# teaghan/sky_embeddings

Measured on AMD Instinct MI355X. Metric: MAE pretrain images/sec (5x64x64, ViT-B), higher is better.
Workload: dtype f16; 1 GPU; mim_32.ini-as-BASELINE configs[1]: MAE ViT-Base/16, 5x64x64, mask_ratio=0.75, bs=256/GPU, AdamW+cosine, norm_pix mse; global_batch=256, parallelism=dp1, rccl_ranks=1, graph=True, adamw_in_wgrad_epilogue=True

## Files before the change

include/skyemb.h:

```cpp
#ifndef SKYEMB_H
#define SKYEMB_H

#include <stdint.h>

#ifdef __cplusplus
extern "C" {
#endif

#define SKYEMB_BF16 0
#define SKYEMB_F32 1
#define SKYEMB_F16 2

#define SKYEMB_KC 0
#define SKYEMB_RC 1

#define SKYEMB_ACT_NONE 0
#define SKYEMB_ACT_GELU 1
#define SKYEMB_ACT_DGELU 2

const char *skyemb_last_error(void);
int skyemb_version(void);
int skyemb_debug_skip(int mask);
#define SKYEMB_GEMM_COUNT_FALLBACK 0
#define SKYEMB_GEMM_COUNT_PIPE 1
// ... 45 lines not shown
    int32_t tile;
    int32_t class_mask;
    int32_t reserved;
} skyemb_gemm_group_info;
int64_t skyemb_gemm_group_blob_bytes(int n);
int skyemb_gemm_group_plan(const skyemb_gemm_args *args, int n, int tile, void *blob_host, int64_t blob_bytes,
                           skyemb_gemm_group_info *info);
int skyemb_gemm_group_launch(const void *blob_dev, const skyemb_gemm_group_info *info, void *stream);
typedef struct skyemb_adamw_desc {
    float *g_base, *p, *m, *v;
    void *p_lp;
    const float *hyper;
    int64_t n_decay;
    float beta1, beta2, eps, weight_decay, grad_scale;
    int32_t enabled;
} skyemb_adamw_desc;
int skyemb_gemm_group_plan_adamw(const skyemb_gemm_args *args, int n, int tile, const skyemb_adamw_desc *adamw, void *blob_host,
                                 int64_t blob_bytes, skyemb_gemm_group_info *info);
int skyemb_gemm_group_plan_side_adamw(const skyemb_gemm_args *args, int n, int tile, const skyemb_adamw_desc *adamw, int own_step,
                                      int64_t side_lo, int64_t side_hi, int side_blocks, void *blob_host, int64_t blob_bytes,
                                      skyemb_gemm_group_info *info);
typedef struct skyemb_ln_bwd_side {
    const void *dy;
    const float *x, *gamma, *mean, *rstd;
    const float *g_in;
    float *g_out;
    void *g_lp;
    float *part;
    int32_t M, D;
} skyemb_ln_bwd_side;
int skyemb_gemm_group_attach_ln_bwd(void *blob_host, int64_t blob_bytes, skyemb_gemm_group_info *info, const skyemb_ln_bwd_side *ln);

int skyemb_colsum(const void *X, int dtype, int64_t ldx, int M, int N, float *out, void *stream);

int skyemb_random_mask_from_noise(const float *noise, int B, int L, int keep, int64_t *ids_restore, float *mask,
                                  int32_t *ids_keep, int32_t *dec_dst, int32_t *dec_tab, int n_extra, void *stream);
int skyemb_simmim_mask_from_noise(const float *noise, const float *ratio_u, double max_ratio, int B, int C, int L, int grid, int p,
                                  float *out_mask, void *stream);

int skyemb_patch_gather(const float *imgs, const float *pmv, const int32_t *ids_keep, void *out, int dtype, int B,
                        int C, int H, int W, int p, int keep, float pixel_mean, float pixel_std, void *stream);

int skyemb_patch_gather_blend(const float *imgs, const float *pmv, const int32_t *ids_keep, const float *pixel_mask, void *out,
                              int dtype, int B, int C, int H, int W, int p, int keep, float pixel_mean, float pixel_std,
                              void *stream);
int skyemb_patch_gather_bwd_pmv_blend(const float *imgs, const int32_t *ids_keep, const float *pixel_mask, const float *drows,
                                      float *partial, float *dpmv, int B, int C, int H, int W, int p, int keep, void *stream);

int skyemb_radec_token_fwd(const float *ra_dec, const float *W0, const float *b0, const float *W1, const float *b1,
                           const float *pos_row, float *x, int64_t row_stride, int B, int D, float *sh, float *z, void *stream);
int skyemb_radec_token_bwd(const float *g, int64_t row_stride, const float *W1, const float *sh, const float *z, float *dz_ws,
                           float *dW0, float *db0, float *dW1, float *db1, int B, int D, void *stream);

int skyemb_patch_gather_bwd_pmv(const float *imgs, const int32_t *ids_keep, const float *drows, float *partial,
                                float *dpmv, int B, int C, int H, int W, int p, int keep, void *stream);

int skyemb_layernorm_fwd(const float *x, const float *gamma, const float *beta, void *y, float *y32, int dtype,
                         float *mean, float *rstd, int M, int D, float eps, void *stream);

int skyemb_layernorm_bwd_blocks(int M);
typedef struct {
    const float *part;
    float *dgamma, *dbeta;
    int32_t nblk, D;
} skyemb_ln_reduce_item;
int skyemb_layernorm_bwd_reduce_batch(const skyemb_ln_reduce_item *items, const int32_t *blocks, int n_blocks, void *stream);
int skyemb_layernorm_bwd(const void *dy, int dy_is_f32, int dtype, const float *x, const float *gamma,
                         const float *mean, const float *rstd, const float *g_in, float *g_out, void *g_lp,
                         float *part, float *dgamma, float *dbeta, int M, int D, void *stream);

#define SKYEMB_MHA_MAX_N 4098
int skyemb_mha_fwd(const void *qkv, void *out, int dtype, int B, int N, int H, int hd, void *stream);
int skyemb_mha_bwd(const void *qkv, const void *dout, void *dqkv, int dtype, int B, int N, int H, int hd,
                   void *stream);
#define SKYEMB_MHA_LDS 0
#define SKYEMB_MHA_STREAM 1
#define SKYEMB_MHA_MFMA_PACKED 2
#define SKYEMB_MHA_MFMA_SINGLE 3
#define SKYEMB_MHA_MFMA_STRIP 4
#define SKYEMB_MHA_MFMA_LONG 5
#define SKYEMB_MHA_SW_NO_MFMA 1
#define SKYEMB_MHA_SW_WPB1 2
#define SKYEMB_MHA_SW_WPB4 4
typedef struct {
    int32_t family;
    int32_t hd;
    int32_t waves;
    int32_t per_wave_floats, nheads;
    int32_t grid_x, grid_y, block;
    int64_t lds_bytes;
    int64_t lds_limit;
} skyemb_mha_plan_t;
int skyemb_mha_plan(int bwd, int dtype, int B, int N, int H, int hd, int switches, skyemb_mha_plan_t *out);

int skyemb_fill_mask_tokens(float *x, const float *mask, const float *mask_token, const float *dec_pos, int B,
                            int L, int Dd, int n_extra, void *stream);
int skyemb_gather_rows(const float *src, const int32_t *idx, float *out, void *out_lp, int dtype, int n_rows,
                       int D, void *stream);
int skyemb_rowsum_select(const float *src, int64_t ld, const float *sel, int row0, int inner, int outer_stride,
                         int n_rows, int D, float *partial, float *out, void *stream);

int skyemb_masked_patch_loss(const float *imgs, const float *pred, const float *mask, float *loss, void *dpred,
                             float *dpred32, int dtype, float *ws, int B, int C, int H, int W, int p, int extra,
                             float pixel_mean, float pixel_std, int norm_pix, int loss_l1, float dscale, void *stream);

int skyemb_simmim_pixel_loss(const float *imgs, const float *pred_tok, const float *pixel_mask, float *loss, void *dpred_tok,
                             int dtype, float *pred_img, float *ws, int B, int C, int H, int W, int p, int extra,
                             float pixel_mean, float pixel_std, int norm_pix, int loss_l1, int pooled, float dscale, void *stream);

int skyemb_set_scalars(float *dst, float a, float b, float c, float d, void *stream);
int skyemb_adamw(float *p, void *g, float *m, float *v, void *p_lp, int dtype, int64_t n, int64_t n_decay,
                 const float *hyper, float lr, float bc1, float bc2, float beta1, float beta2, float eps, float wd,
                 float grad_scale, int zero_grad, int grad_dtype, void *stream);
int skyemb_cast(const float *src, void *dst, int dtype, int64_t n, void *stream);
int skyemb_grad_probe(const void *g, int grad_dtype, int64_t n, uint32_t *state, void *stream);
int skyemb_adamw_guarded(float *p, void *g, float *m, float *v, void *p_lp, int dtype, int64_t n, int64_t n_decay,
                         const float *hyper, float lr, float bc1, float bc2, float beta1, float beta2, float eps, float wd,
                         float grad_scale, int zero_grad, int grad_dtype, const uint32_t *skip, void *stream);
typedef struct skyemb_adamw_group { float lr, bc1, bc2, beta1, beta2, eps, wd; int32_t decayed; } skyemb_adamw_group;
typedef struct skyemb_adamw_segment { int64_t offset, n; int32_t group, reserved; } skyemb_adamw_segment;
typedef struct skyemb_adamw_work { int64_t offset; int32_t n, group; } skyemb_adamw_work;
int skyemb_adamw_segments_limits(int32_t *max_groups, int32_t *chunk_elems, int32_t *max_grid);
int skyemb_adamw_segments_plan(const skyemb_adamw_segment *segs, int n_segs, int n_groups, int64_t buffer_n, void *table_host,
                               int64_t table_bytes, int64_t *need_bytes, int32_t *n_work);
int skyemb_adamw_segments(float *p, const float *g, float *m, float *v, void *p_lp, int dtype, const void *table_dev, int32_t n_work,
                          const skyemb_adamw_group *groups, int n_groups, float grad_scale, const uint32_t *skip, void *stream);

int skyemb_gather_rows_host(const void *src, int64_t row_bytes, const int64_t *idx, int64_t n, int64_t src_rows, void *dst,
                            int nthreads);
int skyemb_h5_unchunk_host(const void *file_base, int64_t file_bytes, const int64_t *chunk_addr, const int64_t *chunk_off,
                           int64_t nchunks, int rank, const int64_t *chunk_dims, const int64_t *dset_dims, int elem_size, void *dst,
                           int nthreads);
int skyemb_fits_decode_tiles_host(int codec, const void *base, int64_t base_bytes, const int64_t *off, const int64_t *len,
                                  const int64_t *npix, const int64_t *dst_off, int64_t ntiles, int bytepix, int blocksize, void *dst,
                                  int64_t dst_pixels, int nthreads);
int skyemb_fits_dequantise_tiles_host(const int32_t *q, const int64_t *q_off, const int64_t *y0, const int64_t *x0, const int64_t *h,
                                      const int64_t *w, const int64_t *table_row, int64_t ntiles, const double *zscale, const double *zzero,
                                      const int32_t *blank, const uint8_t *has_blank, const float *rand, int method, int zdither0,
                                      float *out, int64_t H, int64_t W, int big_endian_out, int nthreads);
int skyemb_tile_cutouts(const void *tile, const int *big_endian, int C, int H, int W, const int *h0, const int *w0, int n, int S,
                        float lo, float hi, int use_lo, int use_hi, float *out, void *stream);
int skyemb_clip_crop(const float *src, float *dst, int64_t n_planes, int Hs, int Ws, int size, float lo, float hi,
                     int use_lo, int use_hi, void *stream);

int skyemb_augment(const float *imgs, float *out, const float *params, const int32_t *nan_mask, const float *noise, int B, int C,
                   int S, int A, void *stream);

int skyemb_standardise(const float *x, const float *mu, const float *sigma, float *out, int64_t N, int D,
                       void *stream);
int skyemb_weighted_norms(const float *x, const float *w, float *norms, float *xw_out, int64_t N, int D,
                          void *stream);
int skyemb_cosine_topk_chunks(int64_t N, int Q, int D, int k);
int skyemb_cosine_topk(const float *tw, const float *qn, const float *bank, const float *xn, int Q, int64_t N,
                       int D, int k, float eps, int64_t idx_offset, int nchunks, const float *thr0, float *part_s,
                       int64_t *part_i, void *stream);
int skyemb_kth_largest_floor(const float *x, int Q, int S, int k, float *out, void *stream);
int skyemb_cosine_sample_floor(const float *tw, const float *qn, const float *sample, const float *sample_norms, int Q, int64_t S,
                               int D, int k, float eps, float *ws, float *floor_out, void *stream);
int skyemb_cosine_sample_floor_applicable(int Q, int64_t S, int D, int k);
int skyemb_topk_merge(const float *in_s, const int64_t *in_i, int Q, int nlists, int k, float *out_s,
                      int64_t *out_i, void *ws, void *stream);

int skyemb_topk_prefilter_applicable(int Q, int64_t N, int D, int k);
int64_t skyemb_topk_prefilter_ws_bytes(int Q, int D, int k);
int skyemb_topk_prefilter_ws_layout(int Q, int D, int k, int64_t *out, int n);
int64_t skyemb_bank16_bytes(int64_t N, int D);
// ... 223 lines not shown
```

sky_embeddings_amd/_lib.py:

```python
from __future__ import annotations

import ctypes
import os
import subprocess

import torch

_HERE = os.path.dirname(os.path.abspath(__file__))
SO_PATH = os.environ.get("SKYEMB_LIB") or os.path.join(_HERE, "libskyemb.so")
CSRC = os.path.join(_HERE, "csrc")

BF16, F32, F16 = 0, 1, 2
ABI_VERSION = 111
KC, RC = 0, 1
ACT_NONE, ACT_GELU, ACT_DGELU = 0, 1, 2
COMBINE_MIN, COMBINE_MEAN, COMBINE_MAX = 0, 1, 2
METRIC_MSE, METRIC_MAE = 1, 2
MHA_LDS, MHA_STREAM, MHA_MFMA_PACKED, MHA_MFMA_SINGLE, MHA_MFMA_STRIP, MHA_MFMA_LONG = range(6)
MHA_SW_NO_MFMA, MHA_SW_WPB1, MHA_SW_WPB4 = 1, 2, 4
PF_ROWS, PF_TOKENS, PF_TOKENS_MEAN = range(3)
PF_BANK_F32, PF_BANK_F16, PF_BANK_BF16 = range(3)
PF_LO_UNSET, PF_MAX_SLICES = 2, 6
PROBE_CHUNKS, PROBE_MAX_F, PROBE_MIN_K, PROBE_MAX_K = 32, 4096, 3, 16


class SkyembLibraryError(RuntimeError):
    pass


class SkyembError(RuntimeError):
    pass


c_i32, c_i64, c_f32, c_vp = ctypes.c_int32, ctypes.c_int64, ctypes.c_float, ctypes.c_void_p
c_f64 = ctypes.c_double


class GemmArgs(ctypes.Structure):
    _fields_ = [
        ("A", c_vp), ("B", c_vp), ("lda", c_i64), ("ldb", c_i64), ("a_layout", c_i32), ("b_layout", c_i32),
        ("M", c_i32), ("N", c_i32), ("K", c_i32), ("dtype", c_i32), ("alpha", c_f32),
        ("bias", c_vp), ("table", c_vp), ("tab_row", c_vp), ("ldt", c_i64), ("dst_row", c_vp),
        ("resid", c_vp), ("ldr", c_i64), ("aux", c_vp), ("ldaux", c_i64), ("act", c_i32),
        ("out_f32", c_vp), ("ldo32", c_i64), ("out", c_vp), ("ldo", c_i64), ("out2", c_vp), ("ldo2", c_i64),
        ("tile", c_i32), ("colsum_a", c_vp), ("ws", c_vp), ("ws_bytes", c_i64), ("split_k", c_i32), ("prefetch_wgs", c_i32),
        ("prefetch", c_vp), ("prefetch_bytes", c_i64),
    ]


class AdamwDesc(ctypes.Structure):
    _fields_ = [("g_base", c_vp), ("p", c_vp), ("m", c_vp), ("v", c_vp), ("p_lp", c_vp), ("hyper", c_vp), ("n_decay", c_i64),
                ("beta1", c_f32), ("beta2", c_f32), ("eps", c_f32), ("weight_decay", c_f32), ("grad_scale", c_f32), ("enabled", c_i32)]


class LnBwdSide(ctypes.Structure):
    _fields_ = [("dy", c_vp), ("x", c_vp), ("gamma", c_vp), ("mean", c_vp), ("rstd", c_vp), ("g_in", c_vp), ("g_out", c_vp), ("g_lp", c_vp),
                ("part", c_vp), ("M", c_i32), ("D", c_i32)]


class MhaPlan(ctypes.Structure):
    _fields_ = [("family", c_i32), ("hd", c_i32), ("waves", c_i32), ("per_wave_floats", c_i32), ("nheads", c_i32),
                ("grid_x", c_i32), ("grid_y", c_i32), ("block", c_i32), ("lds_bytes", c_i64), ("lds_limit", c_i64)]


class PrefilterRequest(ctypes.Structure):
    _fields_ = [("kind", c_i32), ("bank", c_i32), ("Q", c_i32), ("P", c_i32), ("D", c_i32), ("k", c_i32), ("N", c_i64), ("combine", c_i32),
                ("top_t", c_i32), ("has_thr0", c_i32), ("sel", c_i32), ("n_live", c_i32), ("last_live", c_i32), ("direct_sel", c_i32),
                ("lo", c_i32), ("eps", c_f32)]


class PrefilterSlice(ctypes.Structure):
    _fields_ = [("mode", c_i32), ("t0", c_i32), ("t1", c_i32), ("bucket", c_i32), ("tail", c_i32), ("tail_sel", c_i32), ("tail_pos", c_i32),
                ("final", c_i32)]


class PrefilterPlan(ctypes.Structure):
    _fields_ = [("use_lo", c_i32), ("cap", c_i32), ("T", c_i32), ("T_tail", c_i32), ("has_tail", c_i32), ("first", c_i32),
                ("first_rows", c_i32), ("direct_end", c_i32), ("ends", c_i32 * 6), ("sel", c_i32), ("bf", c_i32), ("tok", c_i32),
                ("cnt", c_i32), ("tok_word", c_i32), ("lgp", c_i32), ("fold", c_i32), ("top_t", c_i32), ("q_padded", c_i32),
                ("lds_stage1", c_i32), ("lds_close", c_i32), ("lds_rescore", c_i32), ("lds_stage1_limit", c_i32),
                ("lds_close_limit", c_i32), ("eps_a_f32", c_f32), ("gfac", c_f32), ("eps_a", c_f64), ("rows", c_i64), ("n_slices", c_i32),
                ("slice", PrefilterSlice * 6)]


class AdamwGroup(ctypes.Structure):
    _fields_ = [("lr", c_f32), ("bc1", c_f32), ("bc2", c_f32), ("beta1", c_f32), ("beta2", c_f32), ("eps", c_f32), ("wd", c_f32),
                ("decayed", c_i32)]


class AdamwSegment(ctypes.Structure):
    _fields_ = [("offset", c_i64), ("n", c_i64), ("group", c_i32), ("reserved", c_i32)]


class GemmGroupInfo(ctypes.Structure):
    _fields_ = [("total_blocks", c_i32), ("tile", c_i32), ("class_mask", c_i32), ("reserved", c_i32)]


PROTOTYPES = {
    "skyemb_last_error": (ctypes.c_char_p, []),
    "skyemb_version": (c_i32, []),
    "skyemb_debug_skip": (c_i32, [c_i32]),
    "skyemb_gemm_launch_counts": (c_i32, [c_vp, c_i32, c_i32]),
# ... 216 lines not shown
```

sky_embeddings_amd/csrc/attention.hip:

```cpp
#include "attention_plan.h"
#include "common.h"
#include <stdlib.h>

namespace {

__device__ __forceinline__ float dot4(const float4 a, const float4 b, float acc) {
    acc = fmaf(a.x, b.x, acc);
    acc = fmaf(a.y, b.y, acc);
    acc = fmaf(a.z, b.z, acc);
    return fmaf(a.w, b.w, acc);
}

template <typename T>
__device__ __forceinline__ void load_head(const T *__restrict__ src, int64_t row_stride, float *dst, int N, int hd,
                                          int pitch, float scale, int lane) {
    const int v4 = hd >> 2;
    for (int e = lane; e < N * v4; e += 64) {
        const int n = e / v4, d = (e - n * v4) << 2;
        const float4 x = load4<T>(src + (int64_t)n * row_stride + d);
        *(float4 *)&dst[n * pitch + d] = make_float4(x.x * scale, x.y * scale, x.z * scale, x.w * scale);
    }
}

__device__ __forceinline__ void scores_softmax(const float *qs, const float *k, float *P, int N, int NP, int hd, int pitch,
// ... 211 lines not shown
        for (int c = 0; c < SH_C; ++c) a[c] = 0.f;
        for (int j0 = 0; j0 < N; j0 += 64) {
            const int j = j0 + lane;
            float ds = 0.f;
            if (j < N) {
                const float s = dot_row<T>(ra, kb + (int64_t)j * rs, hd), dp = dot_row<T>(rb, vb + (int64_t)j * rs, hd);
                ds = __expf(s - lse_i) * (dp - d_i);
            }
            sa[lane] = ds;
            __builtin_amdgcn_wave_barrier();
            const int nj = N - j0 < 64 ? N - j0 : 64;
            for (int jj = 0; jj < nj; ++jj) {
                const float dsj = sa[jj];
                const T *kr = kb + (int64_t)(j0 + jj) * rs;
#pragma unroll
                for (int c = 0; c < SH_C; ++c)
                    if (lane + 64 * c < hd) a[c] = fmaf(dsj, to_f32<T>(kr[lane + 64 * c]), a[c]);
            }
            __builtin_amdgcn_wave_barrier();
        }
        T *dq = dqb + (int64_t)i * rs;
#pragma unroll
        for (int c = 0; c < SH_C; ++c)
            if (lane + 64 * c < hd) dq[lane + 64 * c] = from_f32<T>(a[c] * scale);
    }
    __syncthreads();
    for (int j = wave; j < N; j += 4) {
        load_row<T>(ra, kb + (int64_t)j * rs, hd, 1.0f, lane);
        load_row<T>(rb, vb + (int64_t)j * rs, hd, 1.0f, lane);
        __builtin_amdgcn_wave_barrier();
        float ak[SH_C], av[SH_C];
#pragma unroll
        for (int c = 0; c < SH_C; ++c) ak[c] = av[c] = 0.f;
        for (int i0 = 0; i0 < N; i0 += 64) {
            const int i = i0 + lane;
            float p = 0.f, ds = 0.f;
            if (i < N) {
                const float s = dot_row<T>(ra, qb + (int64_t)i * rs, hd) * scale, dp = dot_row<T>(rb, ob + (int64_t)i * D, hd);
                p = __expf(s - lse[i]);
                ds = p * (dp - dsum[i]);
            }
            sa[lane] = p;
            sb[lane] = ds;
            __builtin_amdgcn_wave_barrier();
            const int ni = N - i0 < 64 ? N - i0 : 64;
            for (int ii = 0; ii < ni; ++ii) {
                const float pi = sa[ii], dsi = sb[ii];
                const T *qr = qb + (int64_t)(i0 + ii) * rs, *orow = ob + (int64_t)(i0 + ii) * D;
#pragma unroll
                for (int c = 0; c < SH_C; ++c)
                    if (lane + 64 * c < hd) {
                        ak[c] = fmaf(dsi, to_f32<T>(qr[lane + 64 * c]), ak[c]);
                        av[c] = fmaf(pi, to_f32<T>(orow[lane + 64 * c]), av[c]);
                    }
            }
            __builtin_amdgcn_wave_barrier();
        }
        T *dk = dqb + (int64_t)j * rs + D, *dv = dk + D;
#pragma unroll
        for (int c = 0; c < SH_C; ++c)
            if (lane + 64 * c < hd) {
                dk[lane + 64 * c] = from_f32<T>(ak[c] * scale);
                dv[lane + 64 * c] = from_f32<T>(av[c]);
            }
    }
}

int plan_or_refuse(bool bwd, int dtype, int B, int N, int H, int hd, int switches, skyemb_mha_plan_t *p) {
    const char *who = bwd ? "skyemb_mha_bwd" : "skyemb_mha_fwd";
    switch (sky_mha_plan(bwd, dtype, B, N, H, hd, switches, p)) {
    case MHA_OK: return 0;
    case MHA_BAD_SHAPE: skyemb_set_error("%s: bad shape (head dim must be a multiple of 8)", who); return 1;
    case MHA_TOO_LONG: skyemb_set_error("%s: N = %d tokens, more than the supported %d", who, N, SKYEMB_MHA_MAX_N); return 1;
    default: skyemb_set_error("%s: head dim %d with N = %d tokens: at most %d", who, hd, N, SH_MAXHD); return 1;
    }
}

int env_switches() {
    static const int sw = []() {
        const char *off = getenv("SKYEMB_MHA_MFMA"), *wpb = getenv("SKYEMB_MHA_WPB");
        const int w = wpb ? atoi(wpb) : 0;
        return (off && off[0] == '0' ? SKYEMB_MHA_SW_NO_MFMA : 0) | (w == 1 ? SKYEMB_MHA_SW_WPB1 : w ? SKYEMB_MHA_SW_WPB4 : 0);
    }();
    return sw;
}

template <typename T>
int launch_fp32(const skyemb_mha_plan_t &p, bool bwd, const T *qkv, const T *dout, T *out, int B, int N, int H, int hd,
                hipStream_t st, const char *who) {
    const dim3 grid(p.grid_x, p.grid_y), block(p.block);
    if (p.family == SKYEMB_MHA_STREAM) {
        if (!bwd) hipLaunchKernelGGL(mha_fwd_stream_kernel<T>, grid, block, p.lds_bytes, st, qkv, out, B, N, H, hd);
        else hipLaunchKernelGGL(mha_bwd_stream_kernel<T>, grid, block, p.lds_bytes, st, qkv, dout, out, B, N, H, hd);
        return 0;
    }
    if (p.lds_limit)
        if (const int rc = sky_set_lds_limit(bwd ? (const void *)mha_bwd_kernel<T> : (const void *)mha_fwd_kernel<T>, (int)p.lds_limit, who))
            return rc;
    if (!bwd) hipLaunchKernelGGL(mha_fwd_kernel<T>, grid, block, p.lds_bytes, st, qkv, out, B, N, H, hd, p.waves, p.per_wave_floats);
    else hipLaunchKernelGGL(mha_bwd_kernel<T>, grid, block, p.lds_bytes, st, qkv, dout, out, B, N, H, hd, p.waves, p.per_wave_floats);
    return 0;
}

}

int skyemb_mha_mfma_launch(const skyemb_mha_plan_t &p, bool bwd, const void *qkv, const void *dout, void *out, int dtype, int B, int N,
                           int H, hipStream_t st, const char *who);

static int mha_run(bool bwd, const void *qkv, const void *dout, void *out, int dtype, int B, int N, int H, int hd, void *stream) {
    const char *who = bwd ? "skyemb_mha_bwd" : "skyemb_mha_fwd";
    (void)hipGetLastError();
    skyemb_mha_plan_t p;
    if (const int rc = plan_or_refuse(bwd, dtype, B, N, H, hd, env_switches(), &p)) return rc;
    hipStream_t st = (hipStream_t)stream;
    int rc;
    if (p.family >= SKYEMB_MHA_MFMA_PACKED) rc = skyemb_mha_mfma_launch(p, bwd, qkv, dout, out, dtype, B, N, H, st, who);
    else if (dtype == SKYEMB_BF16) rc = launch_fp32(p, bwd, (const bf16_t *)qkv, (const bf16_t *)dout, (bf16_t *)out, B, N, H, hd, st, who);
    else if (dtype == SKYEMB_F16) rc = launch_fp32(p, bwd, (const f16_t *)qkv, (const f16_t *)dout, (f16_t *)out, B, N, H, hd, st, who);
    else rc = launch_fp32(p, bwd, (const float *)qkv, (const float *)dout, (float *)out, B, N, H, hd, st, who);
    if (rc) return rc;
    SKY_LAUNCH_CHECK(who);
    return 0;
}

extern "C" int skyemb_mha_fwd(const void *qkv, void *out, int dtype, int B, int N, int H, int hd, void *stream) {
    return mha_run(false, qkv, nullptr, out, dtype, B, N, H, hd, stream);
}

extern "C" int skyemb_mha_bwd(const void *qkv, const void *dout, void *dqkv, int dtype, int B, int N, int H, int hd,
                              void *stream) {
    return mha_run(true, qkv, dout, dqkv, dtype, B, N, H, hd, stream);
}

extern "C" int skyemb_mha_plan(int bwd, int dtype, int B, int N, int H, int hd, int switches, skyemb_mha_plan_t *out) {
    if (!out) {
        skyemb_set_error("skyemb_mha_plan: out is NULL");
        return 1;
    }
    return plan_or_refuse(bwd != 0, dtype, B, N, H, hd, switches < 0 ? env_switches() : switches, out);
}
```

sky_embeddings_amd/csrc/attention_mfma.hip:

```cpp
#include "attention_plan.h"
#include "lp_twin.h"

namespace {

typedef __attribute__((ext_vector_type(16))) float f32x16;

__device__ __forceinline__ f32x16 mfma32(lp8 a, lp8 b, f32x16 c) {
    return sky_mfma_32x32x16(a, b, c);
}
__device__ __forceinline__ int pi_row(int s, int g, int e) { return 16 * s + 8 * (e >> 2) + 4 * g + (e & 3); }
__device__ __forceinline__ int acc_row(int reg, int g) { return (reg & 3) + 8 * (reg >> 2) + 4 * g; }

__device__ __forceinline__ lp8 zero8() {
    lp8 z;
#pragma unroll
    for (int e = 0; e < 8; ++e) z[e] = (lp_t)0.0f;
    return z;
}
__device__ __forceinline__ lp8 row_frag(const lp_t *base, int64_t row_stride, int r, int g, int s, int N) {
    return r < N ? *(const lp8 *)(base + (int64_t)r * row_stride + 16 * s + 8 * g) : zero8();
}
__device__ __forceinline__ lp8 pack_regs(const f32x16 &x, int s) {
    lp8 f;
#pragma unroll
    for (int e = 0; e < 8; ++e) f[e] = (lp_t)x[8 * s + e];
    return f;
}

typedef __attribute__((address_space(3))) lp4 lds_lp4_t;
template <int HD>
__device__ __forceinline__ void park_rows(lp_t *tile, const lp8 (&f)[HD / 16], int r, int g) {
#pragma unroll
    for (int s = 0; s < HD / 16; ++s) *(lp8 *)(tile + r * (HD + 8) + 16 * s + 8 * g) = f[s];
}
template <int HD>
__device__ __forceinline__ lp8 tok_frag_lds(const lp_t *tile, int blk, int r, int g, int s) {
    const int i = r & 15, q = i >> 2, p = i & 3;
    const int col0 = 32 * blk + (r & 16) + 4 * p;
    const int t0 = 16 * s + 4 * g;
    const lp4 lo = sky_ds_read_tr16_b64((lds_lp4_t *)(tile + (t0 + q) * (HD + 8) + col0));
    const lp4 hi = sky_ds_read_tr16_b64((lds_lp4_t *)(tile + (t0 + 8 + q) * (HD + 8) + col0));
    lp8 f;
    f[0] = lo[0]; f[1] = lo[1]; f[2] = lo[2]; f[3] = lo[3];
    f[4] = hi[0]; f[5] = hi[1]; f[6] = hi[2]; f[7] = hi[3];
    return f;
}
template <int HD>
__device__ __forceinline__ void store_tile(lp_t *dst_row, const f32x16 &t, int blk, int g, float scale) {
#pragma unroll
    for (int q = 0; q < 4; ++q) {
        const int d0 = 32 * blk + 8 * q + 4 * g;
        if (d0 < HD) store4<lp_t>(dst_row + d0, t[4 * q] * scale, t[4 * q + 1] * scale, t[4 * q + 2] * scale, t[4 * q + 3] * scale);
    }
}

struct PackInfo {
    int b0, h, nrows, inv_n;
};
__device__ __forceinline__ PackInfo pack_of(int head, int B, int N, int H) {
    const int P = N <= 16 ? 32 / N : 1;
    const int pack = head / H;
    PackInfo pi;
    pi.h = head - pack * H;
    pi.b0 = pack * P;
    const int ns = B - pi.b0 < P ? B - pi.b0 : P;
    pi.nrows = ns * N;
    pi.inv_n = (65536 + N - 1) / N;
    return pi;
}
__device__ __forceinline__ int seq_of(int row, const PackInfo &pi) { return (row * pi.inv_n) >> 16; }

template <int HD, int WPB = 4>
__global__ __launch_bounds__(64 * WPB) void mha_fwd_mfma_kernel(const lp_t *__restrict__ qkv, lp_t *__restrict__ out, int B,
                                                           int N, int H, int nheads) {
    constexpr int KS = HD / 16, NB = (HD + 31) / 32;
    __shared__ __attribute__((aligned(16))) lp_t park[WPB][32 * (HD + 8)];
    const int lane = threadIdx.x & 63, wave = threadIdx.x >> 6;
    const int head = blockIdx.x * WPB + wave;
    if (head >= nheads) return;
    const PackInfo pk = pack_of(head, B, N, H);
    const int h = pk.h, NR = pk.nrows;
    const int D = H * HD;
    const int64_t rs = 3 * (int64_t)D;
    const int r = lane & 31, g = lane >> 5;
    const lp_t *qb = qkv + (int64_t)pk.b0 * N * rs + h * HD, *kb = qb + D, *vb = qb + 2 * D;
    const int NS = NR > 16 ? 2 : 1;
    const int my_seq = r < NR ? seq_of(r, pk) : 0;

    lp8 qf[KS], kf[KS], vt[2][NB];
#pragma unroll
    for (int s = 0; s < KS; ++s) {
        qf[s] = row_frag(qb, rs, r, g, s, NR);
        kf[s] = row_frag(kb, rs, r, g, s, NR);
    }
    {
        lp8 vf[KS];
#pragma unroll
        for (int s = 0; s < KS; ++s) vf[s] = row_frag(vb, rs, r, g, s, NR);
        park_rows<HD>(park[wave], vf, r, g);
// ... 74 lines not shown
    park_rows<HD>(park[wave][0], kf, r, g);
    park_rows<HD>(park[wave][1], qf, r, g);
    park_rows<HD>(park[wave][2], of, r, g);
    f32x16 st, sn, dpt, dpn;
#pragma unroll
    for (int e = 0; e < 16; ++e) st[e] = sn[e] = dpt[e] = dpn[e] = 0.f;
#pragma unroll
    for (int s = 0; s < KS; ++s) {
        st = mfma32(kf[s], qf[s], st);
        sn = mfma32(qf[s], kf[s], sn);
        dpt = mfma32(vf[s], of[s], dpt);
        dpn = mfma32(of[s], vf[s], dpn);
    }
    bool same[16];
    float mx = -INFINITY;
#pragma unroll
    for (int e = 0; e < 16; ++e) {
        const int j = acc_row(e, g);
        same[e] = j < NR && seq_of(j, pk) == my_seq;
        st[e] = same[e] ? st[e] * scale : -INFINITY;
        mx = fmaxf(mx, st[e]);
    }
    mx = fmaxf(mx, __shfl_xor(mx, 32));
    float sum = 0.f;
#pragma unroll
    for (int e = 0; e < 16; ++e) {
        st[e] = __expf(st[e] - mx);
        sum += st[e];
    }
    sum += __shfl_xor(sum, 32);
    const float inv = 1.0f / sum;
    float rsum = 0.f;
#pragma unroll
    for (int e = 0; e < 16; ++e) {
        st[e] *= inv;
        rsum = fmaf(st[e], dpt[e], rsum);
    }
    rsum += __shfl_xor(rsum, 32);
#pragma unroll
    for (int e = 0; e < 16; ++e) st[e] *= dpt[e] - rsum;
    if (g == 0) {
        stats[wave][0][r] = mx;
        stats[wave][1][r] = inv;
        stats[wave][2][r] = rsum;
    }
    __builtin_amdgcn_wave_barrier();
    f32x16 pn;
#pragma unroll
    for (int e = 0; e < 16; ++e) {
        const int i = acc_row(e, g);
        const float p = (r < NR && same[e]) ? __expf(sn[e] * scale - stats[wave][0][i]) * stats[wave][1][i] : 0.f;
        pn[e] = p;
        sn[e] = p * (dpn[e] - stats[wave][2][i]);
    }

    lp_t *dq = dqkv + ((int64_t)pk.b0 * N + r) * rs + h * HD, *dk = dq + D, *dv = dq + 2 * D;
    lp8 dst_f[2] = {pack_regs(st, 0), pack_regs(st, 1)};
    lp8 dsn_f[2] = {pack_regs(sn, 0), pack_regs(sn, 1)};
    lp8 pn_f[2] = {pack_regs(pn, 0), pack_regs(pn, 1)};
#pragma unroll
    for (int blk = 0; blk < NB; ++blk) {
        f32x16 tq, tk, tv;
#pragma unroll
        for (int e = 0; e < 16; ++e) tq[e] = tk[e] = tv[e] = 0.f;
#pragma unroll
        for (int s = 0; s < 2; ++s) {
            if (s < NS) {
                const lp8 kt = tok_frag_lds<HD>(park[wave][0], blk, r, g, s);
                const lp8 qt = tok_frag_lds<HD>(park[wave][1], blk, r, g, s);
                const lp8 ot = tok_frag_lds<HD>(park[wave][2], blk, r, g, s);
                tq = mfma32(kt, dst_f[s], tq);
                tk = mfma32(qt, dsn_f[s], tk);
                tv = mfma32(ot, pn_f[s], tv);
            }
        }
        if (r < NR) {
            store_tile<HD>(dq, tq, blk, g, scale);
            store_tile<HD>(dk, tk, blk, g, scale);
            store_tile<HD>(dv, tv, blk, g, 1.0f);
        }
    }
}


constexpr int MAX_NT = MHA_MAX_NT;

__device__ __forceinline__ lp8 row_frag_at(const lp_t *base, int64_t row_stride, int row, int g, int s, int N) {
    return row < N ? *(const lp8 *)(base + (int64_t)row * row_stride + 16 * s + 8 * g) : zero8();
}
__device__ __forceinline__ f32x16 zero16() {
    f32x16 z;
#pragma unroll
    for (int e = 0; e < 16; ++e) z[e] = 0.f;
    return z;
}
template <int HD>
__device__ __forceinline__ void stage_rows(lp_t *tile, const lp_t *base, int64_t row_stride, int N, int rows, int tid, int nthreads) {
    constexpr int PR = HD / 8;
    for (int p = tid; p < rows * PR; p += nthreads) {
        const int row = p / PR, c = p - row * PR;
        *(lp8 *)(tile + row * (HD + 8) + 8 * c) = row < N ? *(const lp8 *)(base + (int64_t)row * row_stride + 8 * c) : zero8();
    }
}
template <int HD, int NT, int NTILES>
__device__ __forceinline__ void stage_tiles(lp_t *const (&tiles)[NTILES], const lp_t *const (&bases)[NTILES],
                                            const int64_t (&strides)[NTILES], int N, int rows, int tid) {
    constexpr int PR = HD / 8, THREADS = 64 * NT;
    constexpr int MAXP = ((32 * NT + 4) * PR + THREADS - 1) / THREADS;
    lp8 v[NTILES][MAXP];
#pragma unroll
    for (int t = 0; t < NTILES; ++t)
#pragma unroll
        for (int i = 0; i < MAXP; ++i) {
            const int p = tid + i * THREADS, row = p / PR, c = p - row * PR;
            const int rc = row < N ? row : N - 1;
            v[t][i] = *(const lp8 *)(bases[t] + (int64_t)rc * strides[t] + 8 * c);
        }
#pragma unroll
    for (int t = 0; t < NTILES; ++t)
#pragma unroll
        for (int i = 0; i < MAXP; ++i) {
            const int p = tid + i * THREADS, row = p / PR, c = p - row * PR;
            if (p < rows * PR) *(lp8 *)(tiles[t] + row * (HD + 8) + 8 * c) = row < N ? v[t][i] : zero8();
        }
}
struct StripRows {
    int n4, zrow;
};
template <int HD>
__device__ __forceinline__ lp8 row_frag_lds(const lp_t *tile, int row, int g, int s, const StripRows &sr) {
    row = row < sr.n4 ? row : sr.zrow;
    return *(const lp8 *)(tile + row * (HD + 8) + 16 * s + 8 * g);
}
template <int HD>
__device__ __forceinline__ lp8 tok_frag_strip(const lp_t *tile, int row0, int blk, int r, int g, int s, const StripRows &sr) {
    const int i = r & 15, q = i >> 2, p = i & 3;
    const int col0 = 32 * blk + (r & 16) + 4 * p;
    int g0 = row0 + 16 * s + 4 * g, g1 = g0 + 8;
    g0 = g0 < sr.n4 ? g0 : sr.zrow;
    g1 = g1 < sr.n4 ? g1 : sr.zrow;
    const lp4 lo = sky_ds_read_tr16_b64((lds_lp4_t *)(tile + (g0 + q) * (HD + 8) + col0));
    const lp4 hi = sky_ds_read_tr16_b64((lds_lp4_t *)(tile + (g1 + q) * (HD + 8) + col0));
    lp8 f;
    f[0] = lo[0]; f[1] = lo[1]; f[2] = lo[2]; f[3] = lo[3];
    f[4] = hi[0]; f[5] = hi[1]; f[6] = hi[2]; f[7] = hi[3];
    return f;
}

extern __shared__ __attribute__((aligned(16))) lp_t strip_lds[];

template <int HD, int NT>
__global__ __launch_bounds__(64 * NT) __attribute__((amdgpu_waves_per_eu(NT <= 3 ? 5 : 3))) void mha_fwd_strip_kernel(const lp_t *__restrict__ qkv, lp_t *__restrict__ out, int B,
                                                                int N, int H) {
    constexpr int KS = HD / 16, NB = (HD + 31) / 32, PITCH = HD + 8;
    const StripRows sr = {(N + 3) & ~3, (N + 3) & ~3};
    const int ROWS = sr.n4 + 4;
    lp_t *kt = strip_lds, *vt = strip_lds + ROWS * PITCH;
    const int lane = threadIdx.x & 63, strip = threadIdx.x >> 6;
    const int b = blockIdx.x / H, h = blockIdx.x - b * H;
    const int D = H * HD;
    const int64_t rs = 3 * (int64_t)D;
    const int r = lane & 31, g = lane >> 5;
    const lp_t *qb = qkv + (int64_t)b * N * rs + h * HD, *kb = qb + D, *vb = qb + 2 * D;
    const int my = 32 * strip + r;
    const float scale = rsqrtf((float)HD);

    lp8 qf[KS];
#pragma unroll
    for (int s = 0; s < KS; ++s) qf[s] = row_frag_at(qb, rs, my, g, s, N);
    {
        lp_t *const tiles[2] = {kt, vt};
        const lp_t *const bases[2] = {kb, vb};
        const int64_t strides[2] = {rs, rs};
        stage_tiles<HD, NT, 2>(tiles, bases, strides, N, ROWS, threadIdx.x);
    }
    __syncthreads();
    f32x16 st[NT];
// ... 399 lines not shown
#pragma unroll
                                for (int blk = 0; blk < NB; ++blk)
                                    tq[blk] = mfma32(tok_frag_lds<HD>(t0 + 32 * t * PITCH, blk, r, g, s), df, tq[blk]);
                            }
                }
            }
            if (walk == 0) {
                lse_i = m + logf(l);
                d_i = dacc / l;
                if (active && g == 0) {
                    lse[my] = lse_i;
                    dsum[my] = d_i;
                }
            }
        }
        if (my < N) {
#pragma unroll
            for (int blk = 0; blk < NB; ++blk) store_tile<HD>(dqb + (int64_t)my * rs, tq[blk], blk, g, scale);
        }
    }
    for (int k0 = 32 * wave; k0 - 32 * wave < N; k0 += 32 * LW) {
        const bool active = k0 < N;
        const int my = k0 + r;
        lp8 kf[KS], vf[KS];
#pragma unroll
        for (int s = 0; s < KS; ++s) {
            kf[s] = row_frag_at(kb, rs, my, g, s, N);
            vf[s] = row_frag_at(vb, rs, my, g, s, N);
        }
        f32x16 tk[NB], tv[NB];
#pragma unroll
        for (int blk = 0; blk < NB; ++blk) {
            tk[blk] = zero16();
            tv[blk] = zero16();
        }
        stg.load(qb, rs, ob, D, 0, N, tid);
        for (int i0 = 0; i0 < N; i0 += LB) {
            __syncthreads();
            stg.store(t0, t1, tid);
            __syncthreads();
            if (i0 + LB < N) stg.load(qb, rs, ob, D, i0 + LB, N, tid);
            if (!active) continue;
#pragma unroll
            for (int t = 0; t < 2; ++t) {
                if (i0 + 32 * t >= N) break;
                f32x16 sn = zero16(), dpn = zero16();
#pragma unroll
                for (int s = 0; s < KS; ++s) {
                    sn = mfma32(tile_row<HD>(t0, 32 * t + r, g, s), kf[s], sn);
                    dpn = mfma32(tile_row<HD>(t1, 32 * t + r, g, s), vf[s], dpn);
                }
#pragma unroll
                for (int e = 0; e < 16; ++e) {
                    const int i = i0 + 32 * t + acc_row(e, g);
                    const bool ok = my < N && i < N;
                    const float p = ok ? __expf(sn[e] * scale - lse[i]) : 0.f;
                    dpn[e] = ok ? p * (dpn[e] - dsum[i]) : 0.f;
                    sn[e] = p;
                }
#pragma unroll
                for (int s = 0; s < 2; ++s) {
                    if (i0 + 32 * t + 16 * s >= N) break;
                    const lp8 pf = pack_regs(sn, s), df = pack_regs(dpn, s);
#pragma unroll
                    for (int blk = 0; blk < NB; ++blk) {
                        tk[blk] = mfma32(tok_frag_lds<HD>(t0 + 32 * t * PITCH, blk, r, g, s), df, tk[blk]);
                        tv[blk] = mfma32(tok_frag_lds<HD>(t1 + 32 * t * PITCH, blk, r, g, s), pf, tv[blk]);
                    }
                }
            }
        }
        if (my < N) {
            lp_t *dk = dqb + (int64_t)my * rs + D, *dv = dk + D;
#pragma unroll
            for (int blk = 0; blk < NB; ++blk) {
                store_tile<HD>(dk, tk[blk], blk, g, scale);
                store_tile<HD>(dv, tv[blk], blk, g, 1.0f);
            }
        }
    }
}

template <int HD, int WPB>
void launch_tile(const skyemb_mha_plan_t &p, bool bwd, const lp_t *x, const lp_t *dout, lp_t *out, int B, int N, int H, hipStream_t st) {
    const dim3 grid(p.grid_x), block(p.block);
    if (!bwd) hipLaunchKernelGGL((mha_fwd_mfma_kernel<HD, WPB>), grid, block, 0, st, x, out, B, N, H, p.nheads);
    else hipLaunchKernelGGL((mha_bwd_mfma_kernel<HD, WPB>), grid, block, 0, st, x, dout, out, B, N, H, p.nheads);
}

template <int HD>
int launch_plan(const skyemb_mha_plan_t &p, bool bwd, const lp_t *x, const lp_t *dout, lp_t *out, int B, int N, int H, hipStream_t st,
                const char *who) {
    if (p.family == SKYEMB_MHA_MFMA_STRIP) {
        if (p.waves == 2) return launch_strip<HD, 2>(p, bwd, x, dout, out, B, N, H, st, who);
        if (p.waves == 3) return launch_strip<HD, 3>(p, bwd, x, dout, out, B, N, H, st, who);
        return launch_strip<HD, 4>(p, bwd, x, dout, out, B, N, H, st, who);
    }
    if (p.family == SKYEMB_MHA_MFMA_LONG) {
        const dim3 grid(p.grid_x, p.grid_y), block(p.block);
        if (!bwd) hipLaunchKernelGGL((mha_fwd_long_kernel<HD>), grid, block, p.lds_bytes, st, x, out, B, N, H);
        else hipLaunchKernelGGL((mha_bwd_long_kernel<HD>), grid, block, p.lds_bytes, st, x, dout, out, B, N, H);
    } else if (p.waves == 1) {
        launch_tile<HD, 1>(p, bwd, x, dout, out, B, N, H, st);
    } else {
        launch_tile<HD, 4>(p, bwd, x, dout, out, B, N, H, st);
    }
    return 0;
}

}

#ifndef SKY_F16
int skyemb_mha_mfma_launch_f16(const skyemb_mha_plan_t &p, bool bwd, const void *qkv, const void *dout, void *out, int dtype, int B, int N,
                               int H, hipStream_t st, const char *who);
#endif
int SKY_TWIN(skyemb_mha_mfma_launch)(const skyemb_mha_plan_t &p, bool bwd, const void *qkv, const void *dout, void *out, int dtype, int B,
                                     int N, int H, hipStream_t st, const char *who) {
#ifndef SKY_F16
    if (dtype == SKYEMB_F16) return skyemb_mha_mfma_launch_f16(p, bwd, qkv, dout, out, dtype, B, N, H, st, who);
#endif
    if (p.hd == 32) return launch_plan<32>(p, bwd, (const lp_t *)qkv, (const lp_t *)dout, (lp_t *)out, B, N, H, st, who);
    return launch_plan<64>(p, bwd, (const lp_t *)qkv, (const lp_t *)dout, (lp_t *)out, B, N, H, st, who);
}
```

Measured before the change: 55170 images/sec.

## Add single-pass short-sequence MHA backward kernel with permlane-widened stores

Adds a new backward attention kernel for short sequences (packed tile family). It computes S and S^T, dP and dP^T in registers via MFMA, so the softmax gradient for both orientations is formed in one pass without recomputation loops. Output tiles are repacked with permlane32_swap into wider 16-byte stores. It becomes the default for the MFMA tile path, and the old kernel is kept behind the SKYEMB_MHA_SHORT_BWD=0 switch. The cost is extra LDS parking and register pressure, and the new numerics path needs validation.

```diff
diff --git a/include/skyemb.h b/include/skyemb.h
--- a/include/skyemb.h
+++ b/include/skyemb.h
@@ -151,6 +151,7 @@
 #define SKYEMB_MHA_SW_NO_MFMA 1
 #define SKYEMB_MHA_SW_WPB1 2
 #define SKYEMB_MHA_SW_WPB4 4
+#define SKYEMB_MHA_SW_BWD_V1 8
 typedef struct {
     int32_t family;
     int32_t hd;
diff --git a/sky_embeddings_amd/_lib.py b/sky_embeddings_amd/_lib.py
--- a/sky_embeddings_amd/_lib.py
+++ b/sky_embeddings_amd/_lib.py
@@ -17,7 +17,7 @@
 COMBINE_MIN, COMBINE_MEAN, COMBINE_MAX = 0, 1, 2
 METRIC_MSE, METRIC_MAE = 1, 2
 MHA_LDS, MHA_STREAM, MHA_MFMA_PACKED, MHA_MFMA_SINGLE, MHA_MFMA_STRIP, MHA_MFMA_LONG = range(6)
-MHA_SW_NO_MFMA, MHA_SW_WPB1, MHA_SW_WPB4 = 1, 2, 4
+MHA_SW_NO_MFMA, MHA_SW_WPB1, MHA_SW_WPB4, MHA_SW_BWD_V1 = 1, 2, 4, 8
 PF_ROWS, PF_TOKENS, PF_TOKENS_MEAN = range(3)
 PF_BANK_F32, PF_BANK_F16, PF_BANK_BF16 = range(3)
 PF_LO_UNSET, PF_MAX_SLICES = 2, 6
diff --git a/sky_embeddings_amd/csrc/attention.hip b/sky_embeddings_amd/csrc/attention.hip
--- a/sky_embeddings_amd/csrc/attention.hip
+++ b/sky_embeddings_amd/csrc/attention.hip
@@ -317,7 +317,8 @@
         const int w = wpb ? atoi(wpb) : 0;
         return (off && off[0] == '0' ? SKYEMB_MHA_SW_NO_MFMA : 0) | (w == 1 ? SKYEMB_MHA_SW_WPB1 : w ? SKYEMB_MHA_SW_WPB4 : 0);
     }();
-    return sw;
+    const char *v1 = getenv("SKYEMB_MHA_SHORT_BWD");
+    return sw | (v1 && v1[0] == '0' ? SKYEMB_MHA_SW_BWD_V1 : 0);
 }
 
 template <typename T>
@@ -339,17 +340,18 @@
 
 }
 
-int skyemb_mha_mfma_launch(const skyemb_mha_plan_t &p, bool bwd, const void *qkv, const void *dout, void *out, int dtype, int B, int N,
-                           int H, hipStream_t st, const char *who);
+int skyemb_mha_mfma_launch(const skyemb_mha_plan_t &p, int switches, bool bwd, const void *qkv, const void *dout, void *out, int dtype, int B,
+                           int N, int H, hipStream_t st, const char *who);
 
 static int mha_run(bool bwd, const void *qkv, const void *dout, void *out, int dtype, int B, int N, int H, int hd, void *stream) {
     const char *who = bwd ? "skyemb_mha_bwd" : "skyemb_mha_fwd";
     (void)hipGetLastError();
     skyemb_mha_plan_t p;
-    if (const int rc = plan_or_refuse(bwd, dtype, B, N, H, hd, env_switches(), &p)) return rc;
+    const int switches = env_switches();
+    if (const int rc = plan_or_refuse(bwd, dtype, B, N, H, hd, switches, &p)) return rc;
     hipStream_t st = (hipStream_t)stream;
     int rc;
-    if (p.family >= SKYEMB_MHA_MFMA_PACKED) rc = skyemb_mha_mfma_launch(p, bwd, qkv, dout, out, dtype, B, N, H, st, who);
+    if (p.family >= SKYEMB_MHA_MFMA_PACKED) rc = skyemb_mha_mfma_launch(p, switches, bwd, qkv, dout, out, dtype, B, N, H, st, who);
     else if (dtype == SKYEMB_BF16) rc = launch_fp32(p, bwd, (const bf16_t *)qkv, (const bf16_t *)dout, (bf16_t *)out, B, N, H, hd, st, who);
     else if (dtype == SKYEMB_F16) rc = launch_fp32(p, bwd, (const f16_t *)qkv, (const f16_t *)dout, (f16_t *)out, B, N, H, hd, st, who);
     else rc = launch_fp32(p, bwd, (const float *)qkv, (const float *)dout, (float *)out, B, N, H, hd, st, who);
diff --git a/sky_embeddings_amd/csrc/attention_mfma.hip b/sky_embeddings_amd/csrc/attention_mfma.hip
--- a/sky_embeddings_amd/csrc/attention_mfma.hip
+++ b/sky_embeddings_amd/csrc/attention_mfma.hip
@@ -15,6 +15,12 @@
     lp8 z;
 #pragma unroll
     for (int e = 0; e < 8; ++e) z[e] = (lp_t)0.0f;
+    return z;
+}
+__device__ __forceinline__ f32x16 zero16() {
+    f32x16 z;
+#pragma unroll
+    for (int e = 0; e < 16; ++e) z[e] = 0.f;
     return z;
 }
 __device__ __forceinline__ lp8 row_frag(const lp_t *base, int64_t row_stride, int r, int g, int s, int N) {
@@ -255,17 +261,199 @@
     }
 }
 
+__device__ __forceinline__ lp8 row_frag_clamped(const lp_t *base, int64_t row_stride, int rc, int g, int s) {
+    return *(const lp8 *)(base + (int64_t)rc * row_stride + 16 * s + 8 * g);
+}
+typedef __attribute__((ext_vector_type(2))) unsigned u32x2;
+typedef __attribute__((ext_vector_type(4))) unsigned u32x4;
+__device__ __forceinline__ void widen_tile(const f32x16 &t, float scale, u32x4 (&out)[2]) {
+#pragma unroll
+    for (int k = 0; k < 2; ++k) {
+        lp4 a, b;
+#pragma unroll
+        for (int e = 0; e < 4; ++e) {
+            a[e] = (lp_t)(t[8 * k + e] * scale);
+            b[e] = (lp_t)(t[8 * k + 4 + e] * scale);
+        }
+        const u32x2 lo = __builtin_bit_cast(u32x2, a), hi = __builtin_bit_cast(u32x2, b);
+        const u32x2 x = __builtin_amdgcn_permlane32_swap(lo[0], hi[0], false, false);
+        const u32x2 y = __builtin_amdgcn_permlane32_swap(lo[1], hi[1], false, false);
+        out[k][0] = x[0]; out[k][1] = y[0]; out[k][2] = x[1]; out[k][3] = y[1];
+    }
+}
+template <int HD>
+__device__ __forceinline__ void store_wide(lp_t *dst_row, const u32x4 (&w)[2], int blk, int g) {
+#pragma unroll
+    for (int k = 0; k < 2; ++k)
+        if (32 * blk + 16 * k < HD) *(u32x4 *)(dst_row + 32 * blk + 16 * k + 8 * g) = w[k];
+}
+
+template <int HD, int WPB = 4>
+__global__ __launch_bounds__(64 * WPB) __attribute__((amdgpu_waves_per_eu(HD == 32 ? 4 : 2))) void mha_bwd_short_kernel(const lp_t *__restrict__ qkv, const lp_t *__restrict__ dout,
+                                                           lp_t *__restrict__ dqkv, int B, int N, int H, int nheads) {
+    constexpr int KS = HD / 16, NB = (HD + 31) / 32;
+    __shared__ __attribute__((aligned(16))) float stats[WPB][3][32];
+    __shared__ __attribute__((aligned(16))) lp_t park[WPB][3][32 * (HD + 8)];
+    const int lane = threadIdx.x & 63, wave = __builtin_amdgcn_readfirstlane(threadIdx.x >> 6);
+    const int head = blockIdx.x * WPB + wave;
+    if (head >= nheads) return;
+    const PackInfo pk = pack_of(head, B, N, H);
+    const int h = pk.h, NR = pk.nrows;
+    const int D = H * HD;
+    const int64_t rs = 3 * (int64_t)D;
+    const int r = lane & 31, g = lane >> 5;
+    const lp_t *qb = qkv + (int64_t)pk.b0 * N * rs + h * HD, *kb = qb + D, *vb = qb + 2 * D;
+    const lp_t *ob = dout + (int64_t)pk.b0 * N * D + h * HD;
+    const bool two = NR > 16;
+    const int NG = (NR + 7) >> 3;
+    const float scale = rsqrtf((float)HD);
+    const bool live = r < NR;
+    const int rc = live ? r : NR - 1;
+    const int lo = live ? seq_of(r, pk) * N : 0;
+    const int len = (lo + N < NR ? lo + N : NR) - lo;
+
+    lp8 qf[KS], kf[KS], vf[KS], of[KS];
+#pragma unroll
+    for (int s = 0; s < KS; ++s) {
+        qf[s] = row_frag_clamped(qb, rs, rc, g, s);
+        kf[s] = row_frag_clamped(kb, rs, rc, g, s);
+        vf[s] = row_frag_clamped(vb, rs, rc, g, s);
+        of[s] = row_frag_clamped(ob, D, rc, g, s);
+    }
+#pragma unroll
+    for (int s = 0; s < KS; ++s) {
+        qf[s] = live ? qf[s] : zero8();
+        kf[s] = live ? kf[s] : zero8();
+        vf[s] = live ? vf[s] : zero8();
+        of[s] = live ? of[s] : zero8();
+    }
+    park_rows<HD>(park[wave][0], kf, r, g);
+    park_rows<HD>(park[wave][1], qf, r, g);
+    park_rows<HD>(park[wave][2], of, r, g);
+    __builtin_amdgcn_wave_barrier();
+    f32x16 st = zero16(), sn = zero16(), dpt = zero16(), dpn = zero16();
+#pragma unroll
+    for (int s = 0; s < KS; ++s) {
+        st = mfma32(kf[s], qf[s], st);
+        sn = mfma32(qf[s], kf[s], sn);
+        dpt = mfma32(vf[s], of[s], dpt);
+        dpn = mfma32(of[s], vf[s], dpn);
+    }
+    lp8 kt0[NB], qt0[NB], ot0[NB], kt1[NB], qt1[NB], ot1[NB];
+    auto read_tok = [&]() {
+#pragma unroll
+        for (int blk = 0; blk < NB; ++blk) {
+            kt0[blk] = tok_frag_lds<HD>(park[wave][0], blk, r, g, 0);
+            qt0[blk] = tok_frag_lds<HD>(park[wave][1], blk, r, g, 0);
+            ot0[blk] = tok_frag_lds<HD>(park[wave][2], blk, r, g, 0);
+        }
+        if (HD == 64 && two) {
+#pragma unroll
+            for (int blk = 0; blk < NB; ++blk) {
+                kt1[blk] = tok_frag_lds<HD>(park[wave][0], blk, r, g, 1);
+                qt1[blk] = tok_frag_lds<HD>(park[wave][1], blk, r, g, 1);
+                ot1[blk] = tok_frag_lds<HD>(park[wave][2], blk, r, g, 1);
+            }
+        }
+    };
+    if (HD == 64) read_tok();
+    bool same[16];
+    float mx = -INFINITY;
+#pragma unroll
+    for (int e = 0; e < 16; ++e) {
+        same[e] = (unsigned)(acc_row(e, g) - lo) < (unsigned)len;
+        st[e] = same[e] ? st[e] * scale : -INFINITY;
+        mx = fmaxf(mx, st[e]);
+    }
+    mx = fmaxf(mx, __shfl_xor(mx, 32));
+#pragma unroll
+    for (int q = 0; q < 4; ++q) {
+        if (q < NG) {
+#pragma unroll
+            for (int e = 4 * q; e < 4 * q + 4; ++e) st[e] = __expf(st[e] - mx);
+        } else {
+#pragma unroll
+            for (int e = 4 * q; e < 4 * q + 4; ++e) st[e] = 0.f;
+        }
+    }
+    float sum = 0.f;
+#pragma unroll
+    for (int e = 0; e < 16; ++e) sum += st[e];
+    sum += __shfl_xor(sum, 32);
+    const float inv = 1.0f / sum;
+    float rsum = 0.f;
+#pragma unroll
+    for (int e = 0; e < 16; ++e) {
+        st[e] *= inv;
+        rsum = fmaf(st[e], dpt[e], rsum);
+    }
+    rsum += __shfl_xor(rsum, 32);
+#pragma unroll
+    for (int e = 0; e < 16; ++e) st[e] *= dpt[e] - rsum;
+    const lp8 dst0 = pack_regs(st, 0), dst1 = pack_regs(st, 1);
+    if (g == 0) {
+        stats[wave][0][r] = mx;
+        stats[wave][1][r] = inv;
+        stats[wave][2][r] = rsum;
+    }
+    __builtin_amdgcn_wave_barrier();
+    f32x16 pn;
+#pragma unroll
+    for (int q = 0; q < 4; ++q) {
+        const f32x4 srs = *(const f32x4 *)&stats[wave][2][8 * q + 4 * g];
+        if (q < NG) {
+            const f32x4 smx = *(const f32x4 *)&stats[wave][0][8 * q + 4 * g], sinv = *(const f32x4 *)&stats[wave][1][8 * q + 4 * g];
+#pragma unroll
+            for (int c = 0; c < 4; ++c) {
+                const int e = 4 * q + c;
+                const float p = __expf(sn[e] * scale - smx[c]) * sinv[c];
+                const bool ok = live & same[e];
+                pn[e] = ok ? p : 0.f;
+            }
+        } else {
+#pragma unroll
+            for (int c = 0; c < 4; ++c) pn[4 * q + c] = 0.f;
+        }
+#pragma unroll
+        for (int c = 0; c < 4; ++c) sn[4 * q + c] = pn[4 * q + c] * (dpn[4 * q + c] - srs[c]);
+    }
+
+    if (HD != 64) read_tok();
+    lp_t *dq = dqkv + ((int64_t)pk.b0 * N + r) * rs + h * HD, *dk = dq + D, *dv = dq + 2 * D;
+    const lp8 dsn0 = pack_regs(sn, 0), dsn1 = pack_regs(sn, 1);
+    const lp8 pn0 = pack_regs(pn, 0), pn1 = pack_regs(pn, 1);
+#pragma unroll
+    for (int blk = 0; blk < NB; ++blk) {
+        f32x16 tq = mfma32(kt0[blk], dst0, zero16());
+        f32x16 tk = mfma32(qt0[blk], dsn0, zero16());
+        f32x16 tv = mfma32(ot0[blk], pn0, zero16());
+        if (two) {
+            if (HD != 64) {
+                kt1[blk] = tok_frag_lds<HD>(park[wave][0], blk, r, g, 1);
+                qt1[blk] = tok_frag_lds<HD>(park[wave][1], blk, r, g, 1);
+                ot1[blk] = tok_frag_lds<HD>(park[wave][2], blk, r, g, 1);
+            }
+            tq = mfma32(kt1[blk], dst1, tq);
+            tk = mfma32(qt1[blk], dsn1, tk);
+            tv = mfma32(ot1[blk], pn1, tv);
+        }
+        u32x4 wq[2], wk[2], wv[2];
+        widen_tile(tq, scale, wq);
+        widen_tile(tk, scale, wk);
+        widen_tile(tv, 1.0f, wv);
+        if (live) {
+            store_wide<HD>(dq, wq, blk, g);
+            store_wide<HD>(dk, wk, blk, g);
+            store_wide<HD>(dv, wv, blk, g);
+        }
+    }
+}
+
 
 constexpr int MAX_NT = MHA_MAX_NT;
 
 __device__ __forceinline__ lp8 row_frag_at(const lp_t *base, int64_t row_stride, int row, int g, int s, int N) {
     return row < N ? *(const lp8 *)(base + (int64_t)row * row_stride + 16 * s + 8 * g) : zero8();
-}
-__device__ __forceinline__ f32x16 zero16() {
-    f32x16 z;
-#pragma unroll
-    for (int e = 0; e < 16; ++e) z[e] = 0.f;
-    return z;
 }
 template <int HD>
 __device__ __forceinline__ void stage_rows(lp_t *tile, const lp_t *base, int64_t row_stride, int N, int rows, int tid, int nthreads) {
@@ -831,15 +1019,17 @@
 }
 
 template <int HD, int WPB>
-void launch_tile(const skyemb_mha_plan_t &p, bool bwd, const lp_t *x, const lp_t *dout, lp_t *out, int B, int N, int H, hipStream_t st) {
+void launch_tile(const skyemb_mha_plan_t &p, int switches, bool bwd, const lp_t *x, const lp_t *dout, lp_t *out, int B, int N, int H,
+                 hipStream_t st) {
     const dim3 grid(p.grid_x), block(p.block);
     if (!bwd) hipLaunchKernelGGL((mha_fwd_mfma_kernel<HD, WPB>), grid, block, 0, st, x, out, B, N, H, p.nheads);
-    else hipLaunchKernelGGL((mha_bwd_mfma_kernel<HD, WPB>), grid, block, 0, st, x, dout, out, B, N, H, p.nheads);
-}
-
-template <int HD>
-int launch_plan(const skyemb_mha_plan_t &p, bool bwd, const lp_t *x, const lp_t *dout, lp_t *out, int B, int N, int H, hipStream_t st,
-                const char *who) {
+    else if (switches & SKYEMB_MHA_SW_BWD_V1) hipLaunchKernelGGL((mha_bwd_mfma_kernel<HD, WPB>), grid, block, 0, st, x, dout, out, B, N, H, p.nheads);
+    else hipLaunchKernelGGL((mha_bwd_short_kernel<HD, WPB>), grid, block, 0, st, x, dout, out, B, N, H, p.nheads);
+}
+
+template <int HD>
+int launch_plan(const skyemb_mha_plan_t &p, int switches, bool bwd, const lp_t *x, const lp_t *dout, lp_t *out, int B, int N, int H,
+                hipStream_t st, const char *who) {
     if (p.family == SKYEMB_MHA_MFMA_STRIP) {
         if (p.waves == 2) return launch_strip<HD, 2>(p, bwd, x, dout, out, B, N, H, st, who);
         if (p.waves == 3) return launch_strip<HD, 3>(p, bwd, x, dout, out, B, N, H, st, who);
@@ -850,9 +1040,9 @@
         if (!bwd) hipLaunchKernelGGL((mha_fwd_long_kernel<HD>), grid, block, p.lds_bytes, st, x, out, B, N, H);
         else hipLaunchKernelGGL((mha_bwd_long_kernel<HD>), grid, block, p.lds_bytes, st, x, dout, out, B, N, H);
     } else if (p.waves == 1) {
-        launch_tile<HD, 1>(p, bwd, x, dout, out, B, N, H, st);
+        launch_tile<HD, 1>(p, switches, bwd, x, dout, out, B, N, H, st);
     } else {
-        launch_tile<HD, 4>(p, bwd, x, dout, out, B, N, H, st);
+        launch_tile<HD, 4>(p, switches, bwd, x, dout, out, B, N, H, st);
     }
     return 0;
 }
@@ -860,14 +1050,14 @@
 }
 
 #ifndef SKY_F16
-int skyemb_mha_mfma_launch_f16(const skyemb_mha_plan_t &p, bool bwd, const void *qkv, const void *dout, void *out, int dtype, int B, int N,
-                               int H, hipStream_t st, const char *who);
+int skyemb_mha_mfma_launch_f16(const skyemb_mha_plan_t &p, int switches, bool bwd, const void *qkv, const void *dout, void *out, int dtype,
+                               int B, int N, int H, hipStream_t st, const char *who);
 #endif
-int SKY_TWIN(skyemb_mha_mfma_launch)(const skyemb_mha_plan_t &p, bool bwd, const void *qkv, const void *dout, void *out, int dtype, int B,
-                                     int N, int H, hipStream_t st, const char *who) {
+int SKY_TWIN(skyemb_mha_mfma_launch)(const skyemb_mha_plan_t &p, int switches, bool bwd, const void *qkv, const void *dout, void *out,
+                                     int dtype, int B, int N, int H, hipStream_t st, const char *who) {
 #ifndef SKY_F16
-    if (dtype == SKYEMB_F16) return skyemb_mha_mfma_launch_f16(p, bwd, qkv, dout, out, dtype, B, N, H, st, who);
+    if (dtype == SKYEMB_F16) return skyemb_mha_mfma_launch_f16(p, switches, bwd, qkv, dout, out, dtype, B, N, H, st, who);
 #endif
-    if (p.hd == 32) return launch_plan<32>(p, bwd, (const lp_t *)qkv, (const lp_t *)dout, (lp_t *)out, B, N, H, st, who);
-    return launch_plan<64>(p, bwd, (const lp_t *)qkv, (const lp_t *)dout, (lp_t *)out, B, N, H, st, who);
-}
+    if (p.hd == 32) return launch_plan<32>(p, switches, bwd, (const lp_t *)qkv, (const lp_t *)dout, (lp_t *)out, B, N, H, st, who);
+    return launch_plan<64>(p, switches, bwd, (const lp_t *)qkv, (const lp_t *)dout, (lp_t *)out, B, N, H, st, who);
+}
```

After: 55610 images/sec (median of 6 runs). No clear change (+0.8%).
